# Zilong-Li/BaseVarC

Measured on AMD Instinct MI355X. Metric: sites/sec at N=1e6 samples; achieved HBM GB/s vs roofline, higher is better.
Workload: dtype f64

## Files before the change

basevarc_amd/csrc/bvc_context.hip:

```cpp
#include <cmath>
#include <cstdlib>
#include <cstring>
#include <mutex>
#include <new>

#include "bvc_ctx.h"

hipError_t sync_streams(bvc_ctx *ctx)
{
    hipError_t first = hipSuccess;
    for (hipStream_t s : streams_of(ctx)) {
        const hipError_t e = hipStreamSynchronize(s);
        if (first == hipSuccess) first = e;
    }
    for (bool &p : ctx->em_pending) p = false;
    return first;
}

int drain_on_error(bvc_ctx *ctx, int code)
{
    (void)sync_streams(ctx);
    (void)hipGetLastError();
    return code;
}
// ... 51 lines not shown
}

void reap_timing(bvc_ctx *ctx, bool all)
{
    size_t kept = 0;
    for (size_t i = 0; i < ctx->ev_pending.size(); ++i) {
        bvc_ctx::Triple &t = ctx->ev_pending[i];
        if (!all && hipEventQuery(t.d) != hipSuccess) { (void)hipGetLastError(); ctx->ev_pending[kept++] = t; continue; }
        float ms1 = 0.f, ms2 = 0.f;
        if (hipEventElapsedTime(&ms1, t.a, t.b) == hipSuccess && hipEventElapsedTime(&ms2, t.c, t.d) == hipSuccess) {
            ctx->prof.hist_ms += ms1; ctx->prof.em_ms += ms2;
            ctx->prof.hist_launches += 1; ctx->prof.em_launches += 1; ctx->prof.sites += t.sites;
        } else {
            (void)hipGetLastError();
        }
        give_back(ctx, t);
    }
    ctx->ev_pending.resize(kept);
}

namespace {
std::mutex g_pinned_mu;
std::vector<std::pair<const char *, size_t>> g_pinned;
}

bool in_pinned(const void *p, size_t n)
{
    std::lock_guard<std::mutex> g(g_pinned_mu);
    const char *c = static_cast<const char *>(p);
    for (auto const &r : g_pinned)
        if (c >= r.first && c + n <= r.first + r.second) return true;
    return false;
}

namespace {
struct Knob {
    const char *key, *env;
    int lo, hi, step, dflt;
    int LaunchState::*member;
    bool takes(int v) const { return v >= lo && v <= hi && (v - lo) % step == 0; }
};
const Knob kKnobs[] = {
    {"em_waves_per_cu", "BVC_EM_WAVES_PER_CU", 0, 32, 1, 0, &LaunchState::em_waves_per_cu},
    {"em_wpb", "BVC_EM_WPB", 1, 4, 3, 4, &LaunchState::em_wpb},
    {"hist_split", "BVC_HIST_SPLIT", 0, 64, 1, 0, &LaunchState::hist_split},
    {"group_pipe", "BVC_GROUP_PIPE", 0, 1, 1, 1, &LaunchState::group_pipe},
    {"group_copies_log2", "BVC_GROUP_LOG2C", -1, 5, 1, -1, &LaunchState::group_log2c},
    {"group_big_lds", "BVC_GROUP_BIG_LDS", 0, 1, 1, 1, &LaunchState::group_big_lds},
    {"group_h16", "BVC_GROUP_H16", 0, 1, 1, 0, &LaunchState::group_h16},
    {"em_streams", "BVC_EM_STREAMS", 0, 3, 1, 0, &LaunchState::em_streams},
    {"em_engine", "BVC_EM_ENGINE", 0, 1, 1, 0, &LaunchState::em_engine},
    {"em_tiny_regions", "BVC_EM_TINY_REGIONS", 0, 1, 1, 0, &LaunchState::em_tiny_regions},
    {"em_prune", "BVC_EM_PRUNE", 0, 1, 1, 1, &LaunchState::em_prune},
    {"csr_scatter_max", "BVC_CSR_SCATTER_MAX", 0, 1 << 30, 1, 64, &LaunchState::csr_scatter_max},
    {"stats_copies_log2", "BVC_STATS_LOG2C", 0, kStatsMaxLog2c, 1, 2, &LaunchState::stats_log2c},
    {"host_chunk_kib", nullptr, 1, 1 << 21, 1, 1 << 19, &LaunchState::host_chunk_kib},
};
}

extern "C" {

const char *bvc_version(void) { return "libbvc 0.3.0 (gfx950)"; }

int bvc_device_count(void)
{
    int n = 0;
    if (hipGetDeviceCount(&n) != hipSuccess) { (void)hipGetLastError(); return 0; }
    int ok = 0;
    for (int d = 0; d < n; ++d) {
        hipDeviceProp_t p;
        if (hipGetDeviceProperties(&p, d) == hipSuccess && std::strncmp(p.gcnArchName, "gfx950", 6) == 0) ++ok;
    }
    return ok;
}

static int env_int(const char *name, int lo, int hi, int dflt)
{
    const char *e = getenv(name);
    if (!e) return dflt;
    const int v = atoi(e);
    return (v >= lo && v <= hi) ? v : dflt;
}

int bvc_create(bvc_ctx **out, int device)
{
    if (!out) return BVC_ERR_ARG;
    *out = nullptr;
    int n = 0;
    if (hipGetDeviceCount(&n) != hipSuccess || n <= 0) { (void)hipGetLastError(); return BVC_ERR_NO_DEVICE; }
    if (device < 0 || device >= n) return BVC_ERR_NO_DEVICE;
    hipDeviceProp_t p;
    if (hipGetDeviceProperties(&p, device) != hipSuccess) return BVC_ERR_DEVICE;
    if (std::strncmp(p.gcnArchName, "gfx950", 6) != 0) return BVC_ERR_NO_DEVICE;
    bvc_ctx *ctx = new (std::nothrow) bvc_ctx();
    if (!ctx) return BVC_ERR_ALLOC;
    ctx->device = device;
#ifdef BVC_DIAG_KNOBS
    if (env_int("BVC_BLOCKING_SYNC", 0, 1, 0)) (void)hipSetDeviceFlags(hipDeviceScheduleBlockingSync);
#endif
    ctx->ls.n_cu = p.multiProcessorCount > 0 ? p.multiProcessorCount : 256;
    for (const Knob &k : kKnobs) {
        const char *e = k.env ? getenv(k.env) : nullptr;
        ctx->ls.*k.member = e && k.takes(atoi(e)) ? atoi(e) : k.dflt;
    }
#ifdef BVC_DIAG_KNOBS
    ctx->ls.dbg_levels = env_int("BVC_DBG_LEVELS", 0, 12, 0);
// ... 214 lines not shown
```

basevarc_amd/csrc/bvc_internal.h:

```cpp
#pragma once
#include <hip/hip_runtime.h>
#include <stdint.h>

#include <vector>

#include "../../include/bvc.h"

namespace bvc {

struct LaunchState {
    int n_cu = 256;
    int em_waves_per_cu = 0;
    int em_wpb = 4;
    int hist_split = 0;
    int host_chunk_kib = 1 << 19;
    int em_streams = 0;
    int group_pipe = 1;
    int group_log2c = -1;
    int group_big_lds = 1;
    int group_h16 = 0;
    int em_engine = 0;
    int em_tiny_regions = 0;
    int csr_scatter_max = 64;
    int em_prune = 1;
    int stats_log2c = 2;
    int dbg_levels = 0;
    mutable uint32_t em_epoch = 0;
    struct RaisedLds { const void *kernel; size_t bytes; };
    mutable std::vector<RaisedLds> lds_raised;
};

inline size_t round256(size_t n) { return (n + 255) / 256 * 256; }

struct Layout {
    uintptr_t base = 0;
    size_t at = 0;
    template <class T> T *take(size_t count, size_t pad = 0)
    {
        T *p = reinterpret_cast<T *>(base + at);
        at += round256(count * sizeof(T) + pad);
        return p;
    }
};

hipError_t raise_lds(const LaunchState &st, const void *kernel, size_t bytes);

struct QualLut {
    double a[128];
    double e[128];
    double e_empty;
    double log_e[128];
    double log_a[128];
};

hipError_t launch_hist_dense(LaunchState &st, hipStream_t stream, int64_t n_sites, int64_t n_samples, int64_t row_stride,
                             const int8_t *bases, const int8_t *quals, const uint8_t *group_of_sample,
                             int n_groups, uint32_t *counts, int split, int64_t *group_scratch = nullptr,
                             uint8_t *hist_of_sample = nullptr);
constexpr int kGroupScratchWords = BVC_MAX_GROUPS + 4;
inline size_t group_redo_offset(int64_t n_samples) { return ((size_t)n_samples + 255) & ~(size_t)255; }
inline size_t group_labels_bytes(int64_t n_samples, int64_t n_sites) { return group_redo_offset(n_samples) + (size_t)n_sites + 256; }
int choose_hist_split(const LaunchState &st, int64_t n_sites, int64_t n_samples);

hipError_t launch_hist_packed(LaunchState &st, hipStream_t stream, int64_t n_sites, int64_t n_samples, int64_t row_stride,
                              const uint8_t *packed, uint32_t *counts, int split);
hipError_t launch_hist_packed_groups(LaunchState &st, hipStream_t stream, int64_t n_sites, int64_t n_samples,
                                     int64_t row_stride, const uint8_t *packed, const uint8_t *group_of_sample, int n_groups,
                                     uint32_t *counts, int64_t *group_scratch, uint8_t *hist_of_sample);
hipError_t launch_pack_dense(hipStream_t stream, int64_t n_sites, int64_t n_samples, int64_t stride_in, const int8_t *bases,
                             const int8_t *quals, int64_t stride_out, uint8_t *packed, unsigned long long *bad);

hipError_t launch_stream_read(hipStream_t stream, const void *src, int64_t bytes, uint32_t *sink);

hipError_t launch_hist_csr(LaunchState &st, hipStream_t stream, int64_t n_sites, const int64_t *offsets,
                           const int8_t *bases, const int8_t *quals, uint32_t *counts);

inline bool uses_item_engine(const LaunchState &st, double min_af) { return st.em_engine != 1 && min_af > 0.0; }
hipError_t launch_lrt(const LaunchState &st, hipStream_t stream, int64_t n_sites, const uint32_t *counts,
                      int64_t hist_stride, const int8_t *ref_base, double min_af, const QualLut *lut,
                      const int8_t *comb, const uint8_t *n_comb, bvc_site_result *results, bool shared = false,
                      int shared_waves_per_cu = 0,
                      void *scratch = nullptr);

size_t em_items_scratch_bytes(int64_t n_sites);
hipError_t launch_lrt_items(const LaunchState &st, hipStream_t stream, int64_t n_sites, int n_groups,
                            const uint32_t *counts, int64_t hist_stride, const int8_t *ref_base, double min_af,
                            const QualLut *lut, const int8_t *comb, const uint8_t *n_comb, bvc_site_result *results,
                            void *scratch, const uint8_t **taken_out, bool shared = false);

hipError_t launch_lrt_groups(const LaunchState &st, hipStream_t stream, int64_t n_sites, int n_groups,
                             const uint32_t *grp_counts, const int8_t *ref_base, double min_af, const QualLut *lut,
                             const bvc_site_result *overall, bvc_group_result *grp_results, bool shared = false,
                             int shared_waves_per_cu = 0, void *scratch = nullptr);
size_t em_group_scratch_bytes(int64_t n_sites, int n_groups);
constexpr int kGroupSharedWavesPerCu = 8;

hipError_t launch_sum_groups(hipStream_t stream, int64_t n_sites, int n_hist, const uint32_t *grp_counts,
                             uint32_t *counts);

hipError_t launch_synth_dense(hipStream_t stream, uint64_t seed, int64_t site0, int64_t n_sites,
                              int64_t n_samples, int64_t row_stride, uint32_t cov_thr16,
                              int8_t *bases, int8_t *quals, int8_t *ref_base);

struct PileupTile {
    const uint8_t *text = nullptr;
    bool bin = false;
    const uint32_t *line_start = nullptr;
    const int32_t *sample0 = nullptr, *n_in_batch = nullptr;
    int32_t n_batches = 0, n_pos = 0;
    int32_t line_stride = 0;
    const int32_t *n_pos_dev = nullptr;
    int64_t n_lines_cap = 0;
    uint32_t *line_words = nullptr;
    uint32_t *status = nullptr;
    int64_t *entry_off = nullptr, *obs_off = nullptr, *totals = nullptr;
    bvc_pileup_entry *entries = nullptr;
    int32_t *samples = nullptr;
    int8_t *obs_base = nullptr, *obs_qual = nullptr;
    const uint8_t *group_of_sample = nullptr;
    int64_t n_samples = 0;
    int32_t n_groups = 0;
    uint8_t *obs_label = nullptr;
    int32_t *tally = nullptr;
    bvc_pileup_indel *indels = nullptr;
    uint32_t indel_cap = 0;
};
struct bvc_pileup_region { uint32_t start, len, left_src, left_len; };
hipError_t launch_region_carry(hipStream_t stream, const uint8_t *old_text, uint8_t *text, const bvc_pileup_region *regions, int32_t n_batches);
hipError_t launch_region_index(hipStream_t stream, const PileupTile &P, const bvc_pileup_region *regions, const uint32_t *seg_base,
                               int64_t n_segments, uint32_t *seg_nl, int32_t *lines, int32_t max_pos);
hipError_t launch_region_ends(hipStream_t stream, const PileupTile &P, uint32_t *ends);
hipError_t launch_indel_text(hipStream_t stream, const PileupTile &P, uint8_t *dst, uint32_t dst_cap, uint32_t *used);
hipError_t launch_called_scan(hipStream_t stream, const PileupTile &P, const bvc_site_result *results, int64_t *called_off);
hipError_t launch_called_gather(hipStream_t stream, const PileupTile &P, const int64_t *called_off, bvc_pileup_entry *out_entries,
                                int32_t *out_samples);
hipError_t launch_pileup_count(hipStream_t stream, const PileupTile &P);
hipError_t launch_pileup_write(hipStream_t stream, const PileupTile &P, uint32_t carry_in);
hipError_t launch_hist_csr_groups(LaunchState &st, hipStream_t stream, int64_t n_sites, const int64_t *offsets, const int8_t *bases,
                                  const int8_t *quals, const int32_t *sample_of_obs, const uint8_t *group_of_sample, int64_t n_samples,
                                  int n_groups, uint32_t *counts);
hipError_t launch_hist_csr_labels(LaunchState &st, hipStream_t stream, int64_t n_sites, const int64_t *offsets, const uint8_t *obs,
// ... 46 lines not shown
```

basevarc_amd/csrc/em_items.hip:

```cpp
#include <algorithm>

#include "bvc_device.h"
#include "bvc_internal.h"
#include "em_common.h"

namespace bvc {
namespace {



constexpr int kTiny = 8, kNarrow = 32, kWide = 48;
template <int CPB> constexpr int site_table_bytes() { return 4 * CPB * 5; }

constexpr int kEmptyQ = 128;

struct FitItem {
    int32_t site;
    uint8_t base[4];
    double f0[4];
    double e_excl;
    double inv_n;
    double ll_excl;
};
static_assert(sizeof(FitItem) == 64, "FitItem layout");
// ... 4 lines not shown
    double ll;
    int32_t passes;
    int32_t pad;
};
static_assert(sizeof(FitOut) == 80, "FitOut layout");

struct ItemSite {
    double lr_alt, chi;
    double base_frq[4];
    double lle[4];
    double lla[4];
    double best_chi, best_lr, best_bp[4];
    int32_t depth[4];
    int32_t passes, fits;
    int32_t item[4];
    uint32_t sets;
    uint32_t blist;
    int8_t n_emit, p_deepest;
    int8_t n;
    int8_t k;
    uint8_t state;
    uint8_t first;
    uint8_t later;
    uint8_t round2;
    int8_t best_i;
};

constexpr int kLists = 2;
constexpr int kRounds = 4;
#ifndef BVC_REGION_SITES
#define BVC_REGION_SITES 8
#endif
constexpr int kRegionSites = BVC_REGION_SITES;
constexpr int kPlaces = 4 * kRegionSites;

__device__ __forceinline__ double single_allele_loglik(const double (&lla)[4], const double (&lle)[4], int b)
{
    double ll = 0.0;
#pragma unroll
    for (int j = 0; j < 4; ++j) ll += j == b ? lla[j] : lle[j];
    return ll;
}

__device__ __forceinline__ int64_t hist_index(int64_t p, int n_groups)
{
    if (n_groups <= 0) return p;
    const uint32_t site = (uint32_t)p / (uint32_t)n_groups;
    return (int64_t)site * (n_groups + 1) + ((uint32_t)p - site * (uint32_t)n_groups);
}

__device__ __forceinline__ int64_t ref_index(int64_t p, int n_groups)
{
    return n_groups > 0 ? (int64_t)((uint32_t)p / (uint32_t)n_groups) : p;
}

__device__ __forceinline__ int list_of(uint32_t pm) { return __popc(pm) >= 3 ? 0 : 1; }

__device__ __forceinline__ uint32_t drop_nibble(uint32_t masks, int c)
{
    const uint32_t low = masks & ((1u << (4 * c)) - 1u);
    return low | ((masks >> (4 * c + 4)) << (4 * c));
}

__device__ __forceinline__ int deepest_position(const int32_t (&depth)[4], uint32_t blist, int n)
{
    int best = 0, best_depth = -1;
#pragma unroll
    for (int p = 0; p < 4; ++p) {
        const int dp = pick4(depth, (int)((blist >> (4 * p)) & 3u));
        if (p < n && dp > best_depth) { best_depth = dp; best = p; }
    }
    return best;
}

__device__ __forceinline__ void count_wanted(uint32_t sets, int n_emit, int (&want)[kLists])
{
    want[0] = want[1] = 0;
#pragma unroll
    for (int c = 0; c < 4; ++c)
        if (c < n_emit) {
            const int l = list_of((sets >> (4 * c)) & 0xFu);
            want[0] += l == 0; want[1] += l == 1;
        }
}

__device__ __forceinline__ uint32_t level_subsets(int n, int p_deepest, int &n_first, uint32_t &later)
{
    int cnt = 0;
    const uint32_t masks = subset_masks(n, n - 1, cnt);
    const int c_last = n - 1 - p_deepest;
    later = (masks >> (4 * c_last)) & 0xFu;
    n_first = cnt - 1;
    return drop_nibble(masks, c_last);
}

template <int CPB>
struct Region {
    ItemSite site[kRegionSites];
    FitItem items[kPlaces];
    FitOut outs[kPlaces];
    int want[kRegionSites][kLists];
    int need;
    int next_slot;
    uint32_t arrive;
    alignas(8) uint8_t tab[kRegionSites][site_table_bytes<CPB>()];
};
// ... 379 lines not shown
        if (__ballot(straddle) != 0) {
            double dl = 0.0;
            const double df = fb - fprev, gp = fma(-4.0, fprev, 1.0);
#pragma unroll
            for (int k = 0; k < kSlots; ++k) {
                const double mo = fma(gp, e[k], fprev);
                const double u = df * fma(-4.0, e[k], 1.0) * rcp_cubic(mo);
                double p = fma(-0.25, u, 1.0 / 3.0);
                p = fma(p, u, -0.5);
                p = fma(p, u, 1.0);
                dl = fma(n[k], fabs(u * p), dl);
            }
            dl = item_sum<ROWS, LOG2G>(dl);
            conv = conv || (straddle && dl < kEmEpsilon);
        }
        const bool stop = !done && (conv || it == kEmIters);
        if (__ballot(stop) != 0) {
            if (stop && sub == 0) {
                FitOut *o = outs + item;
                o->ex[unit] = active ? ex : 0.0;
                o->fl[unit] = fb;
                if (ROWS == 2) o->ex[unit + 2] = 0.0;
                if (unit == 0) { o->passes = it + 1; o->pad = 0; }
            }
            done = done || stop;
            if (__ballot(!done) == 0) break;
        }
        fprev = fb;
        dprev = acc_d;
        fb = ex;
        ++it;
    }
    {
        const double fl = outs[valid ? item : item0].fl[unit];
        const double g = fma(-4.0, fl, 1.0);
        double ll = 0.0;
#pragma unroll
        for (int k = 0; k < kSlots; ++k) {
            ll = fma(n[k], log_pos(fma(g, e[k], fl)), ll);
            if ((k & 3) == 3) __builtin_amdgcn_sched_barrier(0);
        }
        ll = item_sum<ROWS, LOG2G>(ll);
        if (valid && unit == 0 && sub == 0) outs[item].ll = ll + items[item].ll_excl;
    }
}

constexpr int kLog2G4 = 1, kLog2G2 = 2;
template <int CPB> constexpr int log2g4() { return CPB == kTiny ? 0 : kLog2G4; }
template <int CPB> constexpr int log2g2() { return CPB == kTiny ? 1 : kLog2G2; }
constexpr double kPruneSlackAbs = 1.0, kPruneSlackRel = 1e-6;

template <class RegionT>
__device__ __forceinline__ void site_decide(RegionT &R, int ls, int lane, int64_t site, int n_groups, int prune,
                                            const int8_t *__restrict__ ref_base, bvc_site_result *__restrict__ results)
{
    ItemSite S = R.site[ls];
    if (S.state != 1) {
        int zero = 0;
        asm volatile("" : "+v"(zero));
        if (lane == 0) { R.want[ls][0] = zero; R.want[ls][1] = zero; R.site[ls].n_emit = 0; }
        return;
    }
    uint32_t sets = 0;
    int n_emit = 0, p_deepest = 0;
    bool finished = false;

    auto fit_loglik = [&](int idx, double (&ex)[4], int &passes) -> double {
        if (!BVC_LDS_OK(15, idx, kPlaces)) idx = 0;
        const FitOut &o = R.outs[idx];
#pragma unroll
        for (int u = 0; u < 4; ++u) ex[u] = o.ex[u];
        passes = o.passes;
        return o.ll;
    };
    auto by_base = [&](uint32_t pm, const double (&ex)[4], double (&bp)[4]) {
#pragma unroll
        for (int j = 0; j < 4; ++j) bp[j] = 0.0;
        int u = 0;
#pragma unroll
        for (int p = 0; p < 4; ++p)
            if ((pm >> p) & 1u) {
                const int b = (S.blist >> (4 * p)) & 3u;
                const double v = u == 0 ? ex[0] : (u == 1 ? ex[1] : (u == 2 ? ex[2] : ex[3]));
                bp[0] = b == 0 ? v : bp[0]; bp[1] = b == 1 ? v : bp[1];
                bp[2] = b == 2 ? v : bp[2]; bp[3] = b == 3 ? v : bp[3];
                ++u;
            }
    };

    int first_sub = 0;
    if (S.first) {
        double ex[4];
        int passes = 0;
        S.lr_alt = fit_loglik(S.item[0], ex, passes);
        by_base((1u << S.n) - 1u, ex, S.base_frq);
        S.passes += passes; S.fits += 1;
        first_sub = 1;
        S.k = (int8_t)(S.n - 1);
        S.first = 0;
    }
    const int n = S.n, k = S.k;
    bool again = false;
    if (k < 1) {
        finished = true;
    } else if (k >= 2) {
        const int c_last = n - 1 - S.p_deepest;
        int i_min = S.best_i;
// ... 48 lines not shown
        } else {
            S.round2 = 0;
            S.lr_alt = best_lr;
            S.chi = best_chi;
            if (best_chi < kLrtThreshold) {
                int cnt_all = 0;
                const uint32_t pm = (subset_masks(n, k, cnt_all) >> (4 * i_min)) & 0xFu;
                uint32_t nl = 0;
                int nn = 0;
#pragma unroll
                for (int p = 0; p < 4; ++p)
                    if ((pm >> p) & 1u) { nl |= ((S.blist >> (4 * p)) & 3u) << (4 * nn); ++nn; }
                S.blist = nl;
                S.n = (int8_t)k;
#pragma unroll
                for (int j = 0; j < 4; ++j) S.base_frq[j] = best_bp[j];
                S.k = (int8_t)(k - 1);
                S.later = 0;
                if (k - 1 >= 2) {
                    uint32_t later = 0;
                    p_deepest = deepest_position(S.depth, nl, k);
                    sets = level_subsets(k, p_deepest, n_emit, later);
                    S.later = (uint8_t)later;
                }
            } else {
                finished = true;
            }
        }
    }
    if (!finished && !again && S.k == 1) {
        const int b0 = (int)(S.blist & 3u), b1 = (int)((S.blist >> 4) & 3u);
        const double ll0 = single_allele_loglik(S.lla, S.lle, b0), ll1 = single_allele_loglik(S.lla, S.lle, b1);
        const double chi0 = 2.0 * (S.lr_alt - ll0), chi1 = 2.0 * (S.lr_alt - ll1);
        const bool second = chi1 < chi0;
        const double best_chi = second ? chi1 : chi0;
        const int bb = second ? b1 : b0;
        S.passes += 4; S.fits += 2;
        S.lr_alt = second ? ll1 : ll0;
        S.chi = best_chi;
        if (best_chi < kLrtThreshold) {
            S.blist = (uint32_t)bb;
            S.n = 1;
            S.base_frq[0] = bb == 0 ? 1.0 : 0.0; S.base_frq[1] = bb == 1 ? 1.0 : 0.0;
            S.base_frq[2] = bb == 2 ? 1.0 : 0.0; S.base_frq[3] = bb == 3 ? 1.0 : 0.0;
        }
        S.k = 0;
        finished = true;
    }
    S.sets = sets; S.n_emit = (int8_t)n_emit; S.p_deepest = (int8_t)p_deepest;
    int want[kLists];
    count_wanted(sets, n_emit, want);
    if (lane == 0) {
        if (finished) {
            store_record(results + site, S, (int)ref_base[ref_index(site, n_groups)], S.n, S.blist);
            S.state = 2;
        }
        R.site[ls] = S;
        R.want[ls][0] = want[0]; R.want[ls][1] = want[1];
    }
}

struct RegionArgs {
    int64_t n_sites;
    int n_groups;
    const uint32_t *counts;
    int64_t hist_stride;
    const QualLut *lut;
    const int8_t *ref_base;
    double min_af;
    const int8_t *comb;
    const uint8_t *n_comb;
    uint8_t *taken;
    bvc_site_result *results;
    uint32_t *kind_epoch;
    uint32_t epoch;
    int dbg_levels;
    int tiny_regions;
    int prune;
    int64_t region0;
};

__device__ __forceinline__ void wave_sync()
{
    __builtin_amdgcn_fence(__ATOMIC_RELEASE, "workgroup");
    __builtin_amdgcn_wave_barrier();
    __builtin_amdgcn_fence(__ATOMIC_ACQUIRE, "workgroup");
}

__device__ __forceinline__ void load_counts(uint32_t (&c)[8], const uint32_t *__restrict__ counts, int64_t hist_stride, int64_t site,
                                            int n_groups, int lane)
{
    const uint32_t *hist = counts + hist_index(site, n_groups) * hist_stride + (lane >> 4) * 128 + (lane & 15);
#pragma unroll
    for (int lvl = 0; lvl < 8; ++lvl) c[lvl] = hist[16 * lvl];
}

template <int TEAM, class RegionT>
__device__ __forceinline__ void team_sync(RegionT &R, uint32_t &phase, int lane)
{
    if (TEAM == 1) { wave_sync(); return; }
    __builtin_amdgcn_fence(__ATOMIC_RELEASE, "workgroup");
    __builtin_amdgcn_wave_barrier();
    phase += TEAM;
    if (lane == 0) {
        __hip_atomic_fetch_add(&R.arrive, 1u, __ATOMIC_RELEASE, __HIP_MEMORY_SCOPE_WORKGROUP);
        while (__hip_atomic_load(&R.arrive, __ATOMIC_ACQUIRE, __HIP_MEMORY_SCOPE_WORKGROUP) - phase > 0x7FFFFFFFu) __builtin_amdgcn_s_sleep(1);
    }
    __builtin_amdgcn_wave_barrier();
    __builtin_amdgcn_fence(__ATOMIC_ACQUIRE, "workgroup");
}

template <int CPB, int TEAM>
__device__ __forceinline__ void region_body(Region<CPB> *regions, const RegionArgs &A)
{
    const int wave = __builtin_amdgcn_readfirstlane((int)(threadIdx.x >> 6));
    const int teams = (int)(blockDim.x >> 6) / TEAM;
    const int member = wave % TEAM;
    const int lane = threadIdx.x & (kWave - 1);
    Region<CPB> &R = regions[wave / TEAM];
    const int64_t n_sites = A.n_sites;
    const int64_t n_regions = (n_sites + kRegionSites - 1) / kRegionSites;
    if (CPB == kWide && A.kind_epoch[1] != A.epoch) return;
    if (CPB == kTiny && A.kind_epoch[0] != A.epoch) return;
    uint32_t phase = 0;
    if (TEAM > 1) {
        if (member == 0 && lane == 0) R.arrive = 0u;
        __syncthreads();
    }
    const int64_t region = A.region0 + (int64_t)blockIdx.x * teams + wave / TEAM;
    for (bool first = true; region < n_regions && first; first = false) {
        const int64_t site0 = region * kRegionSites;
        if (member == 0 && lane == 0) { R.need = 0; R.next_slot = 0; }
        if (TEAM > 1) team_sync<TEAM>(R, phase, lane);
        int need = 0;
        uint32_t cnext[8];
        if (site0 + member < n_sites) load_counts(cnext, A.counts, A.hist_stride, site0 + member, A.n_groups, lane);
#pragma unroll 1
        for (int ls = member; ls < kRegionSites; ls += TEAM) {
            uint32_t c8[8];
#pragma unroll
            for (int k = 0; k < 8; ++k) c8[k] = cnext[k];
            if (ls + TEAM < kRegionSites && site0 + ls + TEAM < n_sites) load_counts(cnext, A.counts, A.hist_stride, site0 + ls + TEAM, A.n_groups, lane);
            if (site0 + ls < n_sites) {
                need = max(need, site_classes<CPB>(R, ls, lane, site0 + ls, c8, A.lut, A.min_af, A.comb, A.n_comb, A.taken));
            } else if (lane == 0) {
                R.site[ls].state = 2; R.site[ls].n_emit = 0;
                R.want[ls][0] = 0; R.want[ls][1] = 0;
            }
        }
        if (TEAM > 1) {
            if (lane == 0) atomicMax(&R.need, need);
            team_sync<TEAM>(R, phase, lane);
            need = R.need;
        } else {
            wave_sync();
        }
        const int kind = (A.tiny_regions && need <= kTiny) ? kTiny : (need <= kNarrow ? kNarrow : kWide);
        if (CPB == kNarrow && kind != kNarrow && member == 0 && lane == 0) A.kind_epoch[kind == kWide ? 1 : 0] = A.epoch;
        if (kind != CPB) {
            if (TEAM > 1) team_sync<TEAM>(R, phase, lane);
            continue;
        }
        if (member == 0 && lane < kRegionSites && R.site[lane].state == 3) {
            const int64_t site = site0 + lane;
            store_record(A.results + site, R.site[lane], (int)A.ref_base[ref_index(site, A.n_groups)], R.site[lane].n,
                         R.site[lane].blist);
            R.site[lane].state = 2;
        }
        team_sync<TEAM>(R, phase, lane);
        for (int round = 0; round < kRounds && round < (A.dbg_levels >> 1); ++round) {
            int cnt[kLists] = {0, 0};
#pragma unroll
            for (int w = 0; w < kRegionSites; ++w) {
#pragma unroll
                for (int l = 0; l < kLists; ++l) cnt[l] += R.want[w][l];
            }
            if (cnt[0] + cnt[1] == 0) break;
            const int first[kLists] = {0, cnt[0]};
            if (!BVC_LDS_OK(16, cnt[0] + cnt[1], kPlaces + 1)) break;
            if (member == 0) region_emit(R, lane, first);
            team_sync<TEAM>(R, phase, lane);
            constexpr int kPerWave4 = 16 >> log2g4<CPB>(), kPerWave2 = 2 * (16 >> log2g2<CPB>());
            const FitItem *items = R.items;
            FitOut *outs = R.outs;
            const uint8_t *tabs = &R.tab[0][0];
            const double *lut_e = A.lut->e;
            const int w0 = (cnt[0] + kPerWave4 - 1) / kPerWave4, w1 = w0 + (cnt[1] + kPerWave2 - 1) / kPerWave2;
            int slot = 0;
#pragma unroll 1
            for (;;) {
                if (TEAM > 1) {
                    if (lane == 0) slot = atomicAdd(&R.next_slot, 1);
                    slot = __builtin_amdgcn_readfirstlane(slot);
                }
                if (slot >= w1) break;
                if (slot < w0) fit_body<4, log2g4<CPB>(), CPB>(slot * kPerWave4, cnt[0], items, outs, tabs, lut_e);
                else fit_body<2, log2g2<CPB>(), CPB>(cnt[0] + (slot - w0) * kPerWave2, cnt[0] + cnt[1], items, outs, tabs, lut_e);
                if (TEAM == 1) ++slot;
            }
            team_sync<TEAM>(R, phase, lane);
            if (TEAM > 1 && member == 0 && lane == 0) R.next_slot = 0;
            if (round + 1 == (A.dbg_levels >> 1) && (A.dbg_levels & 1)) break;
            int my = lane;
            asm volatile("" : "+v"(my));
            if (member == 0 && my < kRegionSites && site0 + my < n_sites)
                site_decide(R, my, 0, site0 + my, A.n_groups, A.prune, A.ref_base, A.results);
            team_sync<TEAM>(R, phase, lane);
        }
        team_sync<TEAM>(R, phase, lane);
    }
}

#define BVC_OCCUPANCY(n) BVC_WAVES_PER_EU(n, n)
#ifdef BVC_RCP_CHUNK
#define BVC_REGION_WAVES_PER_EU 4
#else
#define BVC_REGION_WAVES_PER_EU 3
#endif
constexpr int kMaxRegionWaves = 4;
#ifndef BVC_REGION_TEAM
#define BVC_REGION_TEAM 2
#endif
constexpr int kTeam = BVC_REGION_TEAM;

template <int CPB>
__global__ __launch_bounds__(64 * kMaxRegionWaves) BVC_OCCUPANCY(CPB == kWide ? 2 : BVC_REGION_WAVES_PER_EU) void region_kernel(RegionArgs A)
{
    BVC_POISON_LDS();
    extern __shared__ __attribute__((aligned(16))) unsigned char region_lds[];
    region_body<CPB, kTeam>(reinterpret_cast<Region<CPB> *>(region_lds), A);
}

}

#ifdef BVC_CHECK_LDS
BVC_DEFINE_DEBUG_READER(debug_read_items)
#endif

struct ItemScratch {
    uint8_t *taken;
    uint32_t *kind_epoch;
};

static ItemScratch item_scratch(Layout &L, int64_t n_sites)
{
    const size_t start = L.at;
    ItemScratch s;
    s.taken = L.take<uint8_t>((size_t)n_sites);
    s.kind_epoch = L.take<uint32_t>(0);
    L.at = start + (size_t)n_sites + 256 + 64;
    return s;
}

size_t em_items_scratch_bytes(int64_t n_sites)
{
    Layout size;
    item_scratch(size, n_sites);
    return size.at;
}

hipError_t launch_lrt_items(const LaunchState &st, hipStream_t stream, int64_t n_sites, int n_groups,
                            const uint32_t *counts, int64_t hist_stride, const int8_t *ref_base, double min_af,
                            const QualLut *lut, const int8_t *comb, const uint8_t *n_comb, bvc_site_result *results,
                            void *scratch, const uint8_t **taken_out, bool shared)
{
    Layout slices{reinterpret_cast<uintptr_t>(scratch)};
    const ItemScratch scr = item_scratch(slices, n_sites);
    uint8_t *taken = scr.taken;
    const int64_t regions = (n_sites + kRegionSites - 1) / kRegionSites;
    int per_cu = 0;
    if (st.em_waves_per_cu > 0) per_cu = st.em_waves_per_cu;
    else if (shared) per_cu = 4;
    constexpr int kMaxTeams = kMaxRegionWaves / kTeam;
    int teams;
    int64_t wgs, per_launch;
    if (per_cu > 0) {
        const int want_teams = std::max(1, per_cu / kTeam);
        teams = std::min(want_teams, kMaxTeams);
        wgs = (regions + teams - 1) / teams;
        per_launch = (int64_t)st.n_cu * ((want_teams + teams - 1) / teams);
    } else {
        teams = (int)std::min<int64_t>(kMaxTeams, std::max<int64_t>(1, (regions + st.n_cu - 1) / st.n_cu));
        wgs = (regions + teams - 1) / teams;
        per_launch = wgs;
    }
    RegionArgs A;
    A.n_sites = n_sites; A.n_groups = n_groups; A.counts = counts; A.hist_stride = hist_stride; A.lut = lut;
    A.ref_base = ref_base; A.min_af = min_af; A.comb = comb; A.n_comb = n_comb; A.taken = taken; A.results = results;
    A.kind_epoch = scr.kind_epoch;
    A.epoch = ++st.em_epoch;
    if (A.epoch == 0) A.epoch = ++st.em_epoch;
    A.dbg_levels = st.dbg_levels > 0 ? st.dbg_levels : 2 * kRounds;
    A.tiny_regions = st.em_tiny_regions;
    A.prune = st.em_prune;
    A.region0 = 0;
    const hipError_t e = raise_lds(st, reinterpret_cast<const void *>(region_kernel<kWide>), kMaxTeams * sizeof(Region<kWide>));
    if (e != hipSuccess) return e;
    const dim3 block(64 * teams * kTeam);
    auto sequence = [&](auto kernel, size_t lds_per_team) {
        for (int64_t w0 = 0; w0 < wgs; w0 += per_launch) {
            A.region0 = w0 * teams;
            hipLaunchKernelGGL(kernel, dim3((unsigned)std::min(per_launch, wgs - w0)), block, teams * lds_per_team, stream, A);
        }
        A.region0 = 0;
    };
    sequence(region_kernel<kNarrow>, sizeof(Region<kNarrow>));
    if (st.em_tiny_regions) sequence(region_kernel<kTiny>, sizeof(Region<kTiny>));
    sequence(region_kernel<kWide>, sizeof(Region<kWide>));
    *taken_out = taken;
    return hipGetLastError();
}

}
```

basevarc_amd/csrc/em_kernel.hip:

```cpp
#include "bvc_device.h"
#include "bvc_internal.h"
#include "em_common.h"

namespace bvc {
namespace {

template <int NS>
struct Slots {
    double n[NS];
    double e[NS];
    double d[NS];
    double yp[NS];
};

struct Freq {
    double fb;
};

constexpr int kDppRor8 = 0x128;
constexpr int kDppRowBcast15 = 0x142;
template <int L> constexpr int dpp_newbcast() { return 0x150 + L; }

struct PassOut {
    double ex_own;
// ... 398 lines not shown
            }
            grp_results[site * n_groups + g] = r;
        }
        wave_lds_sync<WPB>();
    }
}

__global__ void var_qual_kernel(int64_t n_sites, bvc_site_result *__restrict__ results)
{
    BVC_POISON_LDS();
    const int64_t s = (int64_t)blockIdx.x * blockDim.x + threadIdx.x;
    if (s >= n_sites) return;
    if (!results[s].called || results[s].var_qual != kVarQualPending) return;
    const double p = kf_gammaq_dev(0.5, results[s].chi / 2.0);
    double vq = (p != 0.0) ? -10 * log10(p) : 10000.0;
    if (vq == 0) vq = 0.0;
    results[s].var_qual = vq;
}

__global__ void sum_groups_kernel(int64_t total, int n_hist, const uint32_t *__restrict__ grp_counts,
                                  uint32_t *__restrict__ counts)
{
    BVC_POISON_LDS();
    const int64_t i = (int64_t)blockIdx.x * blockDim.x + threadIdx.x;
    if (i >= total) return;
    const int64_t site = i / BVC_NCLASS;
    const int key = (int)(i % BVC_NCLASS);
    uint32_t s = 0;
    for (int h = 0; h < n_hist; ++h) s += grp_counts[(site * n_hist + h) * BVC_NCLASS + key];
    counts[i] = s;
}

__global__ void group_comb_kernel(int64_t n_pseudo, int n_groups, const int8_t *__restrict__ ref_base,
                                  const bvc_site_result *__restrict__ overall, int8_t *__restrict__ comb,
                                  uint8_t *__restrict__ n_comb)
{
    BVC_POISON_LDS();
    const int64_t p = (int64_t)blockIdx.x * blockDim.x + threadIdx.x;
    if (p >= n_pseudo) return;
    const int64_t site = p / n_groups;
    int nc = 0;
    int8_t list[4] = {0, 0, 0, 0};
    if (overall[site].called) {
        const int ref = ref_base[site];
        if ((unsigned)ref < 4u) list[nc++] = (int8_t)ref;
        const int n_alt = overall[site].n_alt;
        for (int i = 0; i < 3; ++i)
            if (i < n_alt) list[nc++] = (int8_t)(overall[site].alt_base[i] & 3);
    }
    for (int c = 0; c < 4; ++c) comb[p * 4 + c] = list[c];
    n_comb[p] = (uint8_t)nc;
}

__global__ void group_records_kernel(int64_t n_pseudo, int n_groups, const bvc_site_result *__restrict__ overall,
                                     const bvc_site_result *__restrict__ pseudo, const uint8_t *__restrict__ taken,
                                     bvc_group_result *__restrict__ grp_results)
{
    BVC_POISON_LDS();
    const int64_t p = (int64_t)blockIdx.x * blockDim.x + threadIdx.x;
    if (p >= n_pseudo || !taken[p]) return;
    const int64_t site = p / n_groups;
    const bvc_site_result t = pseudo[p];
    bvc_group_result r;
    for (int j = 0; j < 4; ++j) r.depth[j] = t.depth[j];
    for (int j = 0; j < 6; ++j) r.pad[j] = 0;
    for (int j = 0; j < 3; ++j) r.af[j] = 0.0;
    r.ran = 0; r.present = 0;
    if (overall[site].called) {
        r.ran = t.depth_total > 0 ? 1 : 0;
        const int n_alt = overall[site].n_alt;
        for (int i = 0; i < 3; ++i)
            if (r.ran && i < n_alt)
                for (int tt = 0; tt < 3; ++tt)
                    if (tt < t.n_alt && t.alt_base[tt] == overall[site].alt_base[i]) { r.af[i] = t.af[tt]; r.present |= (uint8_t)(1u << i); }
    }
    grp_results[p] = r;
}

}

#ifdef BVC_CHECK_LDS
BVC_DEFINE_DEBUG_READER(debug_read_wave_engine)
#endif


static int64_t em_grid_cap(const LaunchState &st, bool shared, int shared_waves_per_cu = 0)
{
    int per_cu = shared ? (shared_waves_per_cu > 0 ? shared_waves_per_cu : 8) : 24;
    if (st.em_waves_per_cu > 0) per_cu = st.em_waves_per_cu;
    return (int64_t)per_cu * st.n_cu;
}

struct SiteKernels {
    template <int NS, int WPB, bool ANY = false> static constexpr auto kernel() { return lrt_kernel<NS, WPB, ANY>; }
};
struct GroupKernels {
    template <int NS, int WPB, bool ANY = false> static constexpr auto kernel() { return lrt_groups_kernel<NS, WPB, ANY>; }
};

template <class Family, int WPB, class... Args>
static void launch_variants(hipStream_t stream, int64_t want_waves, const uint8_t *taken, Args... args)
{
    const dim3 grid((unsigned)((want_waves + WPB - 1) / WPB)), block(64 * WPB);
    if (taken) {
        hipLaunchKernelGGL((Family::template kernel<8, WPB, true>()), grid, block, 0, stream, args...);
        return;
    }
    hipLaunchKernelGGL((Family::template kernel<2, WPB>()), grid, block, 0, stream, args...);
    hipLaunchKernelGGL((Family::template kernel<4, WPB>()), grid, block, 0, stream, args...);
    hipLaunchKernelGGL((Family::template kernel<8, WPB>()), grid, block, 0, stream, args...);
}

template <class Family, class... Args>
static void launch_wave_kernels(const LaunchState &st, hipStream_t stream, int64_t n_work, bool shared, int shared_waves_per_cu,
                                const uint8_t *taken, Args... args)
{
    const int64_t cap = em_grid_cap(st, shared, shared_waves_per_cu);
    const int64_t want_waves = n_work < cap ? n_work : cap;
    if (st.em_wpb == 1) launch_variants<Family, 1>(stream, want_waves, taken, args...);
    else launch_variants<Family, 4>(stream, want_waves, taken, args...);
}

template <class Kernel, class... Args>
static void launch_per_element(Kernel kernel, hipStream_t stream, int64_t n, Args... args)
{
    hipLaunchKernelGGL(kernel, dim3((unsigned)((n + 255) / 256)), dim3(256), 0, stream, n, args...);
}

hipError_t launch_lrt(const LaunchState &st, hipStream_t stream, int64_t n_sites, const uint32_t *counts,
                      int64_t hist_stride, const int8_t *ref_base, double min_af, const QualLut *lut,
                      const int8_t *comb, const uint8_t *n_comb, bvc_site_result *results, bool shared,
                      int shared_waves_per_cu, void *scratch)
{
    if (n_sites <= 0) return hipSuccess;
    const uint8_t *taken = nullptr;
    if (scratch && uses_item_engine(st, min_af)) {
        const hipError_t e = launch_lrt_items(st, stream, n_sites, 0, counts, hist_stride, ref_base, min_af, lut, comb, n_comb,
                                              results, scratch, &taken, shared);
        if (e != hipSuccess) return e;
    }
    launch_wave_kernels<SiteKernels>(st, stream, n_sites, shared, shared_waves_per_cu, taken, n_sites, counts, hist_stride, ref_base,
                                     min_af, lut, comb, n_comb, taken, results);
    launch_per_element(var_qual_kernel, stream, n_sites, results);
    return hipGetLastError();
}

struct GroupScratch {
    int8_t *comb;
    uint8_t *n_comb;
    bvc_site_result *pseudo;
    void *items;
};

static GroupScratch group_scratch(Layout &L, int64_t n_pseudo)
{
    GroupScratch s;
    s.comb = L.take<int8_t>((size_t)n_pseudo * 4);
    s.n_comb = L.take<uint8_t>((size_t)n_pseudo);
    s.pseudo = L.take<bvc_site_result>((size_t)n_pseudo);
    s.items = L.take<char>(0);
    L.at += em_items_scratch_bytes(n_pseudo);
    return s;
}

size_t em_group_scratch_bytes(int64_t n_sites, int n_groups)
{
    Layout size;
    group_scratch(size, n_sites * n_groups);
    return size.at;
}

hipError_t launch_lrt_groups(const LaunchState &st, hipStream_t stream, int64_t n_sites, int n_groups,
                             const uint32_t *grp_counts, const int8_t *ref_base, double min_af, const QualLut *lut,
                             const bvc_site_result *overall, bvc_group_result *grp_results, bool shared,
                             int shared_waves_per_cu, void *scratch)
{
    if (n_sites <= 0 || n_groups <= 0) return hipSuccess;
    const int64_t n_work = n_sites * n_groups;
    const uint8_t *taken = nullptr;
    if (scratch && uses_item_engine(st, min_af)) {
        Layout slices{reinterpret_cast<uintptr_t>(scratch)};
        const GroupScratch s = group_scratch(slices, n_work);
        launch_per_element(group_comb_kernel, stream, n_work, n_groups, ref_base, overall, s.comb, s.n_comb);
        const hipError_t e = launch_lrt_items(st, stream, n_work, n_groups, grp_counts, BVC_NCLASS, ref_base, min_af, lut, s.comb,
                                              s.n_comb, s.pseudo, s.items, &taken, shared);
        if (e != hipSuccess) return e;
        launch_per_element(group_records_kernel, stream, n_work, n_groups, overall, s.pseudo, taken, grp_results);
    }
    launch_wave_kernels<GroupKernels>(st, stream, n_work, shared, shared_waves_per_cu, taken, n_sites, n_groups, grp_counts, ref_base,
                                      min_af, lut, overall, taken, grp_results);
    return hipGetLastError();
}

hipError_t launch_sum_groups(hipStream_t stream, int64_t n_sites, int n_hist, const uint32_t *grp_counts,
                             uint32_t *counts)
{
    const int64_t total = n_sites * BVC_NCLASS;
    if (total <= 0) return hipSuccess;
    launch_per_element(sum_groups_kernel, stream, total, n_hist, grp_counts, counts);
    return hipGetLastError();
}

}
```

Baseline: 3.363 million.

## Compact group EM work to called sites before running the item engine

Adds a single-block pack kernel that ballot-compacts the sites called in the overall pass, then builds comb lists and a source map covering only those sites' groups. The item EM engine reads counts through the map and exits early beyond a device-side live count, so per-group EM work on uncalled sites is skipped. A new records kernel fills uncalled sites with depth-only results computed from the histograms. This removes wasted EM work on non-variant sites, at the cost of a serial single-block prefix scan over all sites and a one-shot launch of every wide-region workgroup.

```diff
diff --git a/basevarc_amd/csrc/bvc_context.hip b/basevarc_amd/csrc/bvc_context.hip
--- a/basevarc_amd/csrc/bvc_context.hip
+++ b/basevarc_amd/csrc/bvc_context.hip
@@ -127,6 +127,7 @@
     {"em_engine", "BVC_EM_ENGINE", 0, 1, 1, 0, &LaunchState::em_engine},
     {"em_tiny_regions", "BVC_EM_TINY_REGIONS", 0, 1, 1, 0, &LaunchState::em_tiny_regions},
     {"em_prune", "BVC_EM_PRUNE", 0, 1, 1, 1, &LaunchState::em_prune},
+    {"group_pack", "BVC_GROUP_PACK", 0, 1, 1, 1, &LaunchState::group_pack},
     {"csr_scatter_max", "BVC_CSR_SCATTER_MAX", 0, 1 << 30, 1, 64, &LaunchState::csr_scatter_max},
     {"stats_copies_log2", "BVC_STATS_LOG2C", 0, kStatsMaxLog2c, 1, 2, &LaunchState::stats_log2c},
     {"host_chunk_kib", nullptr, 1, 1 << 21, 1, 1 << 19, &LaunchState::host_chunk_kib},
diff --git a/basevarc_amd/csrc/bvc_internal.h b/basevarc_amd/csrc/bvc_internal.h
--- a/basevarc_amd/csrc/bvc_internal.h
+++ b/basevarc_amd/csrc/bvc_internal.h
@@ -24,6 +24,7 @@
     int csr_scatter_max = 64;
     int em_prune = 1;
     int stats_log2c = 2;
+    int group_pack = 1;
     int dbg_levels = 0;
     mutable uint32_t em_epoch = 0;
     struct RaisedLds { const void *kernel; size_t bytes; };
@@ -86,7 +87,8 @@
 hipError_t launch_lrt_items(const LaunchState &st, hipStream_t stream, int64_t n_sites, int n_groups,
                             const uint32_t *counts, int64_t hist_stride, const int8_t *ref_base, double min_af,
                             const QualLut *lut, const int8_t *comb, const uint8_t *n_comb, bvc_site_result *results,
-                            void *scratch, const uint8_t **taken_out, bool shared = false);
+                            void *scratch, const uint8_t **taken_out, bool shared = false,
+                            const int32_t *site_map = nullptr, const int32_t *n_sites_dev = nullptr);
 
 hipError_t launch_lrt_groups(const LaunchState &st, hipStream_t stream, int64_t n_sites, int n_groups,
                              const uint32_t *grp_counts, const int8_t *ref_base, double min_af, const QualLut *lut,
diff --git a/basevarc_amd/csrc/em_items.hip b/basevarc_amd/csrc/em_items.hip
--- a/basevarc_amd/csrc/em_items.hip
+++ b/basevarc_amd/csrc/em_items.hip
@@ -80,6 +80,11 @@
 __device__ __forceinline__ int64_t ref_index(int64_t p, int n_groups)
 {
     return n_groups > 0 ? (int64_t)((uint32_t)p / (uint32_t)n_groups) : p;
+}
+
+__device__ __forceinline__ int64_t mapped_site(const int32_t *__restrict__ site_map, int64_t j)
+{
+    return site_map ? (int64_t)site_map[j] : j;
 }
 
 __device__ __forceinline__ int list_of(uint32_t pm) { return __popc(pm) >= 3 ? 0 : 1; }
@@ -565,7 +570,8 @@
 
 template <class RegionT>
 __device__ __forceinline__ void site_decide(RegionT &R, int ls, int lane, int64_t site, int n_groups, int prune,
-                                            const int8_t *__restrict__ ref_base, bvc_site_result *__restrict__ results)
+                                            const int32_t *__restrict__ site_map, const int8_t *__restrict__ ref_base,
+                                            bvc_site_result *__restrict__ results)
 {
     ItemSite S = R.site[ls];
     if (S.state != 1) {
@@ -720,7 +726,7 @@
     count_wanted(sets, n_emit, want);
     if (lane == 0) {
         if (finished) {
-            store_record(results + site, S, (int)ref_base[ref_index(site, n_groups)], S.n, S.blist);
+            store_record(results + site, S, (int)ref_base[ref_index(mapped_site(site_map, site), n_groups)], S.n, S.blist);
             S.state = 2;
         }
         R.site[ls] = S;
@@ -746,6 +752,8 @@
     int tiny_regions;
     int prune;
     int64_t region0;
+    const int32_t *site_map;
+    const int32_t *n_sites_dev;
 };
 
 __device__ __forceinline__ void wave_sync()
@@ -786,10 +794,15 @@
     const int member = wave % TEAM;
     const int lane = threadIdx.x & (kWave - 1);
     Region<CPB> &R = regions[wave / TEAM];
-    const int64_t n_sites = A.n_sites;
-    const int64_t n_regions = (n_sites + kRegionSites - 1) / kRegionSites;
     if (CPB == kWide && A.kind_epoch[1] != A.epoch) return;
     if (CPB == kTiny && A.kind_epoch[0] != A.epoch) return;
+    int64_t n_sites = A.n_sites;
+    if (A.n_sites_dev) {
+        const int64_t in_use = *A.n_sites_dev;
+        if (in_use < n_sites) n_sites = in_use;
+        if ((A.region0 + (int64_t)blockIdx.x * teams) * kRegionSites >= n_sites) return;
+    }
+    const int64_t n_regions = (n_sites + kRegionSites - 1) / kRegionSites;
     uint32_t phase = 0;
     if (TEAM > 1) {
         if (member == 0 && lane == 0) R.arrive = 0u;
@@ -802,13 +815,14 @@
         if (TEAM > 1) team_sync<TEAM>(R, phase, lane);
         int need = 0;
         uint32_t cnext[8];
-        if (site0 + member < n_sites) load_counts(cnext, A.counts, A.hist_stride, site0 + member, A.n_groups, lane);
+        if (site0 + member < n_sites) load_counts(cnext, A.counts, A.hist_stride, mapped_site(A.site_map, site0 + member), A.n_groups, lane);
 #pragma unroll 1
         for (int ls = member; ls < kRegionSites; ls += TEAM) {
             uint32_t c8[8];
 #pragma unroll
             for (int k = 0; k < 8; ++k) c8[k] = cnext[k];
-            if (ls + TEAM < kRegionSites && site0 + ls + TEAM < n_sites) load_counts(cnext, A.counts, A.hist_stride, site0 + ls + TEAM, A.n_groups, lane);
+            if (ls + TEAM < kRegionSites && site0 + ls + TEAM < n_sites)
+                load_counts(cnext, A.counts, A.hist_stride, mapped_site(A.site_map, site0 + ls + TEAM), A.n_groups, lane);
             if (site0 + ls < n_sites) {
                 need = max(need, site_classes<CPB>(R, ls, lane, site0 + ls, c8, A.lut, A.min_af, A.comb, A.n_comb, A.taken));
             } else if (lane == 0) {
@@ -831,8 +845,8 @@
         }
         if (member == 0 && lane < kRegionSites && R.site[lane].state == 3) {
             const int64_t site = site0 + lane;
-            store_record(A.results + site, R.site[lane], (int)A.ref_base[ref_index(site, A.n_groups)], R.site[lane].n,
-                         R.site[lane].blist);
+            store_record(A.results + site, R.site[lane], (int)A.ref_base[ref_index(mapped_site(A.site_map, site), A.n_groups)],
+                         R.site[lane].n, R.site[lane].blist);
             R.site[lane].state = 2;
         }
         team_sync<TEAM>(R, phase, lane);
@@ -872,7 +886,7 @@
             int my = lane;
             asm volatile("" : "+v"(my));
             if (member == 0 && my < kRegionSites && site0 + my < n_sites)
-                site_decide(R, my, 0, site0 + my, A.n_groups, A.prune, A.ref_base, A.results);
+                site_decide(R, my, 0, site0 + my, A.n_groups, A.prune, A.site_map, A.ref_base, A.results);
             team_sync<TEAM>(R, phase, lane);
         }
         team_sync<TEAM>(R, phase, lane);
@@ -930,7 +944,8 @@
 hipError_t launch_lrt_items(const LaunchState &st, hipStream_t stream, int64_t n_sites, int n_groups,
                             const uint32_t *counts, int64_t hist_stride, const int8_t *ref_base, double min_af,
                             const QualLut *lut, const int8_t *comb, const uint8_t *n_comb, bvc_site_result *results,
-                            void *scratch, const uint8_t **taken_out, bool shared)
+                            void *scratch, const uint8_t **taken_out, bool shared, const int32_t *site_map,
+                            const int32_t *n_sites_dev)
 {
     Layout slices{reinterpret_cast<uintptr_t>(scratch)};
     const ItemScratch scr = item_scratch(slices, n_sites);
@@ -938,7 +953,7 @@
     const int64_t regions = (n_sites + kRegionSites - 1) / kRegionSites;
     int per_cu = 0;
     if (st.em_waves_per_cu > 0) per_cu = st.em_waves_per_cu;
-    else if (shared) per_cu = 4;
+    else if (shared) per_cu = n_sites_dev ? 2 : 4;
     constexpr int kMaxTeams = kMaxRegionWaves / kTeam;
     int teams;
     int64_t wgs, per_launch;
@@ -962,19 +977,21 @@
     A.tiny_regions = st.em_tiny_regions;
     A.prune = st.em_prune;
     A.region0 = 0;
+    A.site_map = site_map; A.n_sites_dev = n_sites_dev;
     const hipError_t e = raise_lds(st, reinterpret_cast<const void *>(region_kernel<kWide>), kMaxTeams * sizeof(Region<kWide>));
     if (e != hipSuccess) return e;
     const dim3 block(64 * teams * kTeam);
-    auto sequence = [&](auto kernel, size_t lds_per_team) {
-        for (int64_t w0 = 0; w0 < wgs; w0 += per_launch) {
+    auto sequence = [&](auto kernel, size_t lds_per_team, bool one_launch = false) {
+        const int64_t step = one_launch ? wgs : per_launch;
+        for (int64_t w0 = 0; w0 < wgs; w0 += step) {
             A.region0 = w0 * teams;
-            hipLaunchKernelGGL(kernel, dim3((unsigned)std::min(per_launch, wgs - w0)), block, teams * lds_per_team, stream, A);
+            hipLaunchKernelGGL(kernel, dim3((unsigned)std::min(step, wgs - w0)), block, teams * lds_per_team, stream, A);
         }
         A.region0 = 0;
     };
     sequence(region_kernel<kNarrow>, sizeof(Region<kNarrow>));
     if (st.em_tiny_regions) sequence(region_kernel<kTiny>, sizeof(Region<kTiny>));
-    sequence(region_kernel<kWide>, sizeof(Region<kWide>));
+    sequence(region_kernel<kWide>, sizeof(Region<kWide>), n_sites_dev != nullptr);
     *taken_out = taken;
     return hipGetLastError();
 }
diff --git a/basevarc_amd/csrc/em_kernel.hip b/basevarc_amd/csrc/em_kernel.hip
--- a/basevarc_amd/csrc/em_kernel.hip
+++ b/basevarc_amd/csrc/em_kernel.hip
@@ -474,29 +474,115 @@
     n_comb[p] = (uint8_t)nc;
 }
 
-__global__ void group_records_kernel(int64_t n_pseudo, int n_groups, const bvc_site_result *__restrict__ overall,
-                                     const bvc_site_result *__restrict__ pseudo, const uint8_t *__restrict__ taken,
-                                     bvc_group_result *__restrict__ grp_results)
-{
-    BVC_POISON_LDS();
-    const int64_t p = (int64_t)blockIdx.x * blockDim.x + threadIdx.x;
-    if (p >= n_pseudo || !taken[p]) return;
-    const int64_t site = p / n_groups;
-    const bvc_site_result t = pseudo[p];
+__device__ __forceinline__ bvc_group_result group_record_of(const bvc_site_result &t, const bvc_site_result &ov)
+{
     bvc_group_result r;
     for (int j = 0; j < 4; ++j) r.depth[j] = t.depth[j];
     for (int j = 0; j < 6; ++j) r.pad[j] = 0;
     for (int j = 0; j < 3; ++j) r.af[j] = 0.0;
     r.ran = 0; r.present = 0;
-    if (overall[site].called) {
+    if (ov.called) {
         r.ran = t.depth_total > 0 ? 1 : 0;
-        const int n_alt = overall[site].n_alt;
+        const int n_alt = ov.n_alt;
         for (int i = 0; i < 3; ++i)
             if (r.ran && i < n_alt)
                 for (int tt = 0; tt < 3; ++tt)
-                    if (tt < t.n_alt && t.alt_base[tt] == overall[site].alt_base[i]) { r.af[i] = t.af[tt]; r.present |= (uint8_t)(1u << i); }
-    }
-    grp_results[p] = r;
+                    if (tt < t.n_alt && t.alt_base[tt] == ov.alt_base[i]) { r.af[i] = t.af[tt]; r.present |= (uint8_t)(1u << i); }
+    }
+    return r;
+}
+
+__global__ void group_records_kernel(int64_t n_pseudo, int n_groups, const bvc_site_result *__restrict__ overall,
+                                     const bvc_site_result *__restrict__ pseudo, const uint8_t *__restrict__ taken,
+                                     bvc_group_result *__restrict__ grp_results)
+{
+    BVC_POISON_LDS();
+    const int64_t p = (int64_t)blockIdx.x * blockDim.x + threadIdx.x;
+    if (p >= n_pseudo || !taken[p]) return;
+    grp_results[p] = group_record_of(pseudo[p], overall[p / n_groups]);
+}
+
+constexpr int kPackThreads = 1024;
+
+__global__ __launch_bounds__(kPackThreads) void group_pack_kernel(int64_t n_sites, int n_groups, const int8_t *__restrict__ ref_base,
+                                                                  const bvc_site_result *__restrict__ overall, int32_t *called_site,
+                                                                  int32_t *__restrict__ place_of_site, int32_t *__restrict__ n_live,
+                                                                  int32_t *__restrict__ src, int8_t *__restrict__ comb,
+                                                                  uint8_t *__restrict__ n_comb)
+{
+    BVC_POISON_LDS();
+    __shared__ int s_wave[kPackThreads / 64];
+    __shared__ int s_called;
+    const int lane = threadIdx.x & 63, wave = threadIdx.x >> 6;
+    if (threadIdx.x == 0) s_called = 0;
+    __syncthreads();
+    for (int64_t site0 = 0; site0 < n_sites; site0 += kPackThreads) {
+        const int64_t site = site0 + threadIdx.x;
+        const bool called = site < n_sites && overall[site].called;
+        const uint64_t votes = __ballot(called);
+        if (lane == 0) s_wave[wave] = __popcll(votes);
+        __syncthreads();
+        int rank = s_called;
+        for (int w = 0; w < wave; ++w) rank += s_wave[w];
+        rank += __popcll(votes & ((1ull << lane) - 1ull));
+        if (called) called_site[rank] = (int32_t)site;
+        if (site < n_sites) place_of_site[site] = called ? rank * n_groups : -1;
+        __syncthreads();
+        if (threadIdx.x == kPackThreads - 1) s_called = rank + (called ? 1 : 0);
+        __syncthreads();
+    }
+    const int64_t live = (int64_t)s_called * n_groups;
+    if (threadIdx.x == 0) *n_live = (int32_t)live;
+    for (int64_t j = threadIdx.x; j < live; j += kPackThreads) {
+        const int32_t rank = (int32_t)((uint32_t)j / (uint32_t)n_groups);
+        const int64_t site = called_site[rank];
+        const bvc_site_result ov = overall[site];
+        const int ref = ref_base[site];
+        int nc = 0;
+        int8_t list[4] = {0, 0, 0, 0};
+        if ((unsigned)ref < 4u) list[nc++] = (int8_t)ref;
+        for (int i = 0; i < 3; ++i)
+            if (i < ov.n_alt) list[nc++] = (int8_t)(ov.alt_base[i] & 3);
+        src[j] = (int32_t)(site * n_groups + (j - (int64_t)rank * n_groups));
+        for (int c = 0; c < 4; ++c) comb[j * 4 + c] = list[c];
+        n_comb[j] = (uint8_t)nc;
+    }
+}
+
+__global__ __launch_bounds__(256) void group_records_packed_kernel(int64_t n_pseudo, int n_groups, const uint32_t *__restrict__ grp_counts,
+                                                                   const bvc_site_result *__restrict__ overall,
+                                                                   const int32_t *__restrict__ place_of_site,
+                                                                   const bvc_site_result *__restrict__ pseudo,
+                                                                   const uint8_t *__restrict__ taken, uint8_t *__restrict__ taken_orig,
+                                                                   bvc_group_result *__restrict__ grp_results)
+{
+    BVC_POISON_LDS();
+    const int64_t p = (int64_t)blockIdx.x * 4 + __builtin_amdgcn_readfirstlane((int)(threadIdx.x >> 6));
+    if (p >= n_pseudo) return;
+    const int lane = threadIdx.x & 63;
+    const int64_t site = p / n_groups;
+    const int g = (int)(p - site * n_groups);
+    const int32_t place0 = place_of_site[site];
+    if (place0 < 0) {
+        const uint32_t *hist = grp_counts + (site * (n_groups + 1) + g) * BVC_NCLASS;
+        const int row = lane >> 4, t = lane & 15;
+        int d = 0;
+#pragma unroll
+        for (int lvl = 0; lvl < 8; ++lvl) d += (int)hist[row * 128 + t + 16 * lvl];
+        d = row_sum(d);
+        const int d0 = __builtin_amdgcn_readlane(d, 0), d1 = __builtin_amdgcn_readlane(d, 16);
+        const int d2 = __builtin_amdgcn_readlane(d, 32), d3 = __builtin_amdgcn_readlane(d, 48);
+        if (lane == 0) {
+            grp_results[p] = group_record_depths(d0, d1, d2, d3);
+            taken_orig[p] = 1;
+        }
+        return;
+    }
+    if (lane != 0) return;
+    const int64_t j = (int64_t)place0 + g;
+    const uint8_t mine = taken[j];
+    taken_orig[p] = mine;
+    if (mine) grp_results[p] = group_record_of(pseudo[j], overall[site]);
 }
 
 }
@@ -571,15 +657,26 @@
     int8_t *comb;
     uint8_t *n_comb;
     bvc_site_result *pseudo;
+    int32_t *src;
+    int32_t *called_site;
+    int32_t *place_of_site;
+    int32_t *n_live;
+    uint8_t *taken_orig;
     void *items;
 };
 
-static GroupScratch group_scratch(Layout &L, int64_t n_pseudo)
-{
+static GroupScratch group_scratch(Layout &L, int64_t n_sites, int n_groups)
+{
+    const int64_t n_pseudo = n_sites * n_groups;
     GroupScratch s;
     s.comb = L.take<int8_t>((size_t)n_pseudo * 4);
     s.n_comb = L.take<uint8_t>((size_t)n_pseudo);
     s.pseudo = L.take<bvc_site_result>((size_t)n_pseudo);
+    s.src = L.take<int32_t>((size_t)n_pseudo);
+    s.called_site = L.take<int32_t>((size_t)n_sites);
+    s.place_of_site = L.take<int32_t>((size_t)n_sites);
+    s.n_live = L.take<int32_t>(1);
+    s.taken_orig = L.take<uint8_t>((size_t)n_pseudo);
     s.items = L.take<char>(0);
     L.at += em_items_scratch_bytes(n_pseudo);
     return s;
@@ -588,7 +685,7 @@
 size_t em_group_scratch_bytes(int64_t n_sites, int n_groups)
 {
     Layout size;
-    group_scratch(size, n_sites * n_groups);
+    group_scratch(size, n_sites, n_groups);
     return size.at;
 }
 
@@ -602,12 +699,23 @@
     const uint8_t *taken = nullptr;
     if (scratch && uses_item_engine(st, min_af)) {
         Layout slices{reinterpret_cast<uintptr_t>(scratch)};
-        const GroupScratch s = group_scratch(slices, n_work);
-        launch_per_element(group_comb_kernel, stream, n_work, n_groups, ref_base, overall, s.comb, s.n_comb);
-        const hipError_t e = launch_lrt_items(st, stream, n_work, n_groups, grp_counts, BVC_NCLASS, ref_base, min_af, lut, s.comb,
-                                              s.n_comb, s.pseudo, s.items, &taken, shared);
-        if (e != hipSuccess) return e;
-        launch_per_element(group_records_kernel, stream, n_work, n_groups, overall, s.pseudo, taken, grp_results);
+        const GroupScratch s = group_scratch(slices, n_sites, n_groups);
+        if (st.group_pack) {
+            hipLaunchKernelGGL(group_pack_kernel, dim3(1), dim3(kPackThreads), 0, stream, n_sites, n_groups, ref_base, overall,
+                               s.called_site, s.place_of_site, s.n_live, s.src, s.comb, s.n_comb);
+            const hipError_t e = launch_lrt_items(st, stream, n_work, n_groups, grp_counts, BVC_NCLASS, ref_base, min_af, lut, s.comb,
+                                                  s.n_comb, s.pseudo, s.items, &taken, shared, s.src, s.n_live);
+            if (e != hipSuccess) return e;
+            hipLaunchKernelGGL(group_records_packed_kernel, dim3((unsigned)((n_work + 3) / 4)), dim3(256), 0, stream, n_work, n_groups,
+                               grp_counts, overall, s.place_of_site, s.pseudo, taken, s.taken_orig, grp_results);
+            taken = s.taken_orig;
+        } else {
+            launch_per_element(group_comb_kernel, stream, n_work, n_groups, ref_base, overall, s.comb, s.n_comb);
+            const hipError_t e = launch_lrt_items(st, stream, n_work, n_groups, grp_counts, BVC_NCLASS, ref_base, min_af, lut, s.comb,
+                                                  s.n_comb, s.pseudo, s.items, &taken, shared);
+            if (e != hipSuccess) return e;
+            launch_per_element(group_records_kernel, stream, n_work, n_groups, overall, s.pseudo, taken, grp_results);
+        }
     }
     launch_wave_kernels<GroupKernels>(st, stream, n_work, shared, shared_waves_per_cu, taken, n_sites, n_groups, grp_counts, ref_base,
                                       min_af, lut, overall, taken, grp_results);
```

Result: no change. 3.361 million (median of 2 runs) (-0.1%).
